# RmSchaffert/ACCV-Lab

Measured on AMD Instinct MI355X. Metric: heatmap frames/sec (1920x1080 fp32, ragged N_obj in [1,128], fused clear+draw), higher is better.
Workload: dtype f32

## Files before the change

accv-lab_amd/csrc/draw_heatmap.hip:

```cpp
#include <hip/hip_runtime.h>
#include <hip/hip_ext.h>

#include <algorithm>
#include <atomic>
#include <climits>
#include <cstdint>
#include <cstring>
#include <type_traits>

#include "accv_common.h"
#include "polyline_arith.h"

namespace {

constexpr int kWavesPerGroup = 1;
constexpr int kBoxTileR = 8;
constexpr int kCand = 64;
constexpr float kLog2e = 1.4426950408889634f;

struct SplatParams {
    float* hm;
    const int32_t* centers;
    const int32_t* radii;
    const int32_t* labels;
    const void* counts;
    const int32_t* plane_off;
    int H, W;
    int n_max;
    int n_classes;
    int tiles_x, tiles_y;
    long long n_tiles;
    float factor, k;
    int counts_i64;
    int grid3d;
    float dense_area;
    const float* centers_f;
    const float* boxes_f;
    float stride;
    int radius, n_groups;
};

constexpr int kMaxScales = 4;
struct MultiParams {
    SplatParams scale[kMaxScales];
    long long tile_begin[kMaxScales + 1];
    int n_scales;
};

struct __attribute__((aligned(16))) Hit {
    int x, y;
    float c2;
    unsigned box;
};

template <int PX>
struct Vec;
typedef float vfloat4 __attribute__((ext_vector_type(4)));
template <>
struct Vec<4> {
    using type = vfloat4;
};
template <>
struct Vec<1> {
    using type = float;
};

__device__ __forceinline__ float raw_exp2(float x) { return __builtin_amdgcn_exp2f(x); }

__device__ __forceinline__ float max_skip_nan(float acc, float v)
{
    float r;
    asm("v_max_f32 %0, %1, %2" : "=v"(r) : "v"(acc), "v"(v));
    return r;
}

struct TileCtx {
    int tx0, ty0, tx1, ty1;
    long long plane;
    const int2* centers2;
    const int32_t* radii;
    const int32_t* labels;
    const float2* centers_f;
    const float4* boxes_f;
    float4 box0;
    float stride;
    int radius;
    int n, cls;
};

template <bool SCALAR_COUNT = false>
__device__ __forceinline__ void plane_objects(const SplatParams& p, TileCtx& t);

template <int TW, int TH, int WPG, bool SCALAR_COUNT = false>
__device__ __forceinline__ bool locate_tile(const SplatParams& p, int wave, TileCtx& t, long long linear_group)
{
    int tx, ty;
    if (p.grid3d) {
        tx = blockIdx.x * WPG + wave;
        ty = blockIdx.y;
        t.plane = blockIdx.z;
        if (tx >= p.tiles_x) return false;
    } else {
        const long long tile = linear_group * WPG + wave;
        if (tile >= p.n_tiles) return false;
        if (p.n_tiles <= 0x7fffffffll) {
            const unsigned t32 = (unsigned)tile, t2 = t32 / (unsigned)p.tiles_x;
            tx = (int)(t32 - t2 * (unsigned)p.tiles_x);
            const unsigned pl = t2 / (unsigned)p.tiles_y;
            ty = (int)(t2 - pl * (unsigned)p.tiles_y);
            t.plane = pl;
        } else {
            tx = (int)(tile % p.tiles_x);
            const long long t2 = tile / p.tiles_x;
            ty = (int)(t2 % p.tiles_y);
            t.plane = t2 / p.tiles_y;
        }
    }
    t.tx0 = tx * TW;
    t.ty0 = ty * TH;
    t.tx1 = min(t.tx0 + TW, p.W);
    t.ty1 = min(t.ty0 + TH, p.H);
    plane_objects<SCALAR_COUNT>(p, t);
    return true;
}

template <bool SCALAR_COUNT>
__device__ __forceinline__ void plane_objects(const SplatParams& p, TileCtx& t)
{
    long long obj_base;
    t.cls = -1;
    if (p.plane_off) {
        const int o0 = p.plane_off[t.plane];
        obj_base = o0;
        t.n = p.plane_off[t.plane + 1] - o0;
    } else {
        long long s = t.plane;
        if (p.n_classes > 0) {
            s = t.plane / p.n_classes;
            t.cls = (int)(t.plane - s * p.n_classes);
        }
        long long cnt;
        if constexpr (SCALAR_COUNT) {
            if (p.n_groups > 0)
                t.box0 = reinterpret_cast<const float4*>(p.boxes_f)[t.plane * p.n_groups + min((int)(threadIdx.x & 63), p.n_groups - 1)];
            using ConstI32 = const __attribute__((address_space(4))) int;
            using ConstI64 = const __attribute__((address_space(4))) long long;
            const uintptr_t base = reinterpret_cast<uintptr_t>(p.counts);
            cnt = p.counts_i64 ? reinterpret_cast<ConstI64*>(base)[s] : (long long)reinterpret_cast<ConstI32*>(base)[s];
        } else {
            cnt = p.counts_i64 ? ((const long long*)p.counts)[s] : (long long)((const int*)p.counts)[s];
        }
        t.n = (int)max(0ll, min(cnt, (long long)p.n_max));
        obj_base = s * p.n_max;
    }
    t.centers2 = reinterpret_cast<const int2*>(p.centers) + obj_base;
    t.radii = p.radii + obj_base;
    t.labels = p.labels + obj_base;
    t.centers_f = reinterpret_cast<const float2*>(p.centers_f) + obj_base;
    t.boxes_f = reinterpret_cast<const float4*>(p.boxes_f) + (p.n_groups > 0 ? (t.plane * p.n_groups) : obj_base);
    t.stride = p.stride;
    t.radius = p.radius;
}

struct Cand {
    int x, y, r, label;
};
template <int SRC = 0>
__device__ __forceinline__ Cand cull_load(const TileCtx& t, int base, int lane)
{
    const int cc = min(base + lane, t.n - 1);
    if constexpr (SRC == 1) {
        const float2 c = t.centers_f[cc];
        const float4 b = t.boxes_f[cc];
        const float m = fminf(fminf(c.x - b.x, c.y - b.y), fminf(b.z - c.x, b.w - c.y));
        const bool pow2 = (__float_as_uint(t.stride) & 0x007fffffu) == 0u && t.stride > 1.0e-30f && t.stride < 1.0e30f;
        if (pow2) {
            const float inv = 1.0f / t.stride;
            int r = (int)ceilf(m * inv);
            if (r < 1) r = 1;
            return Cand{(int)(c.x * inv), (int)(c.y * inv), r, 0};
        }
        int r = (int)ceilf(__fdiv_rn(m, t.stride));
        if (r < 1) r = 1;
        return Cand{(int)__fdiv_rn(c.x, t.stride), (int)__fdiv_rn(c.y, t.stride), r, 0};
    } else if constexpr (SRC == 2) {
        const float2 c = t.centers_f[cc];
        const bool bad = (c.x != c.x) || (c.y != c.y);
        if (bad) return Cand{0, 0, -1, 0};
        return Cand{(int)__fdiv_rn(c.x, t.stride), (int)__fdiv_rn(c.y, t.stride), t.radius, 0};
    } else {
        const int2 cxy = t.centers2[cc];
        return Cand{cxy.x, cxy.y, t.radii[cc], t.labels[cc]};
    }
}
__device__ __forceinline__ unsigned long long cull_test(const TileCtx& t, int base, int lane, const Cand& c)
{
    constexpr int kClampXY = 1 << 29, kClampR = 1 << 30;
    const int xc = min(max(c.x, -kClampXY), kClampXY), yc = min(max(c.y, -kClampXY), kClampXY);
    const int rc = min(c.r, kClampR);
    const bool hit = (base + lane < t.n) && (t.cls < 0 || c.label == t.cls) && c.r >= 0 && xc - rc < t.tx1 &&
                     xc + rc >= t.tx0 && yc - rc < t.ty1 && yc + rc >= t.ty0;
    return __ballot(hit);
}
template <int SRC = 0>
__device__ __forceinline__ unsigned long long cull_round(const TileCtx& t, int base, int lane, int& x, int& y, int& r)
{
    const Cand c = cull_load<SRC>(t, base, lane);
    x = c.x;
    y = c.y;
    r = c.r;
    return cull_test(t, base, lane, c);
}

__device__ __forceinline__ float hit_exponent_scale(const SplatParams& p, int r)
{
    const float sigma = (float)(2 * r + 1) / p.factor;
    return kLog2e / (2.0f * sigma * sigma);
}
__device__ __forceinline__ Hit make_hit(const SplatParams& p, const TileCtx& t, int x, int y, int r, float c2);
__device__ __forceinline__ Hit make_hit(const SplatParams& p, const TileCtx& t, int x, int y, int r)
{
    return make_hit(p, t, x, y, r, hit_exponent_scale(p, r));
}
__device__ __forceinline__ Hit make_hit(const SplatParams& p, const TileCtx& t, int x, int y, int r, float c2)
{
    const long long x0 = (long long)x - min(x, r), x1 = (long long)x + min((long long)p.W - x, (long long)r + 1);
    const long long y0 = (long long)y - min(y, r), y1 = (long long)y + min((long long)p.H - y, (long long)r + 1);
    const long long xlo = max(x0, (long long)t.tx0) - t.tx0, xhi = min(x1, (long long)t.tx1) - t.tx0;
    const long long ylo = max(y0, (long long)t.ty0) - t.ty0, yhi = min(y1, (long long)t.ty1) - t.ty0;
    unsigned box = 0;
    if (xhi > xlo && yhi > ylo) box = (unsigned)xlo | ((unsigned)xhi << 8) | ((unsigned)ylo << 16) | ((unsigned)yhi << 24);
    return Hit{x, y, c2, box};
}

__device__ __forceinline__ float max3_skip_nan(float acc, float a, float b)
{
    float r;
    asm("v_max3_f32 %0, %1, %2, %3" : "=v"(r) : "v"(acc), "v"(a), "v"(b));
    return r;
}

template <int PX, int R, bool CLEAR, int SM, int WPG, int SRC>
__device__ __forceinline__ void splat_body(const SplatParams& p, long long linear_group)
{
    constexpr int kWavesPerGroup = WPG;
    constexpr int TW = 32 * PX;
    constexpr int TH = 2 * R;
    static_assert(R % 4 == 0, "row registers are fetched four at a time");

    __shared__ Hit s_hit[kWavesPerGroup][kCand];
    __shared__ __attribute__((aligned(16))) float s_ey[kWavesPerGroup][kCand][TH];

    const int lane = threadIdx.x & 63;
    const int wave = __builtin_amdgcn_readfirstlane(threadIdx.x >> 6);
    TileCtx t;
    if (!locate_tile<TW, TH, kWavesPerGroup>(p, wave, t, linear_group)) return;
    const int tx0 = t.tx0, ty0 = t.ty0, n = t.n;
    const long long plane = t.plane;

    const int sub = lane >> 5;
    const int col0 = tx0 + (lane & 31) * PX;

    float acc[R][PX];
    const float init = CLEAR ? 0.0f : __builtin_nanf("");
#pragma unroll
    for (int i = 0; i < R; ++i)
#pragma unroll
        for (int c = 0; c < PX; ++c) acc[i][c] = init;

    int total_hits = 0;
    float cover = 0.0f;

    for (int base = 0; base < n; base += kCand) {
        int x, y, r;
        const unsigned long long m = cull_round<SRC>(t, base, lane, x, y, r);
        if constexpr (SM == 5) {
            const float dia = (float)(2 * min(max(r, 0), 1 << 20) + 1);
            cover += (base + lane < n) ? dia * dia : 0.0f;
        }
        const bool hit = (m >> lane) & 1ull;
        const int nh = __popcll(m);
        if (nh == 0) continue;
        if constexpr (!CLEAR) {
            if (total_hits == 0 && col0 < p.W) {
                const float* plane_rd = p.hm + (size_t)plane * (size_t)p.H * (size_t)p.W;
#pragma unroll
                for (int i = 0; i < R; ++i) {
                    const int row = ty0 + sub * R + i;
                    if (row < p.H) {
                        if constexpr (PX == 4) {
                            const vfloat4 o = *reinterpret_cast<const vfloat4*>(plane_rd + (size_t)row * p.W + col0);
                            acc[i][0] = o.x;
                            acc[i][1] = o.y;
                            acc[i][2] = o.z;
                            acc[i][3] = o.w;
                        } else {
                            acc[i][0] = plane_rd[(size_t)row * p.W + col0];
                        }
                    }
                }
            }
        }
        if (hit) s_hit[wave][__popcll(m & ((1ull << lane) - 1ull))] = make_hit(p, t, x, y, r);
        __builtin_amdgcn_fence(__ATOMIC_RELEASE, "wavefront");
        __builtin_amdgcn_fence(__ATOMIC_ACQUIRE, "wavefront");

        for (int t = lane; t < nh * TH; t += 64) {
            const int h = t / TH, rr = t % TH;
            const Hit hy = s_hit[wave][h];
            const float d = (float)(ty0 + rr - hy.y);
            const float v = p.k * raw_exp2(-(d * d) * hy.c2);
            const unsigned ylo = (hy.box >> 16) & 255u, yhi = hy.box >> 24;
            s_ey[wave][h][rr] = ((unsigned)rr >= ylo && (unsigned)rr < yhi) ? v : __builtin_nanf("");
        }
        __builtin_amdgcn_fence(__ATOMIC_RELEASE, "wavefront");
        __builtin_amdgcn_fence(__ATOMIC_ACQUIRE, "wavefront");

        const unsigned colr0 = (unsigned)(lane & 31) * PX;
        auto column_factors = [&](const Hit& hx, float (&ex)[PX]) {
            const unsigned xlo = hx.box & 255u, xhi = (hx.box >> 8) & 255u;
#pragma unroll
            for (int c = 0; c < PX; ++c) {
                const float d = (float)(col0 + c - hx.x);
                const float e = raw_exp2(-(d * d) * hx.c2);
                ex[c] = (colr0 + c >= xlo && colr0 + c < xhi) ? e : __builtin_nanf("");
            }
        };
        int h = 0;
        for (; CLEAR && h + 1 < nh; h += 2) {
            float exa[PX], exb[PX];
            column_factors(s_hit[wave][h], exa);
            column_factors(s_hit[wave][h + 1], exb);
#pragma unroll
            for (int q = 0; q < R / 4; ++q) {
                const float4 a4 = *reinterpret_cast<const float4*>(&s_ey[wave][h][sub * R + 4 * q]);
                const float4 b4 = *reinterpret_cast<const float4*>(&s_ey[wave][h + 1][sub * R + 4 * q]);
                const float eya[4] = {a4.x, a4.y, a4.z, a4.w}, eyb[4] = {b4.x, b4.y, b4.z, b4.w};
#pragma unroll
                for (int i = 0; i < 4; ++i)
#pragma unroll
                    for (int c = 0; c < PX; ++c)
                        acc[4 * q + i][c] = max3_skip_nan(acc[4 * q + i][c], exa[c] * eya[i], exb[c] * eyb[i]);
            }
        }
        for (; h < nh; ++h) {
            float ex[PX];
            column_factors(s_hit[wave][h], ex);
#pragma unroll
            for (int q = 0; q < R / 4; ++q) {
                const float4 e4 = *reinterpret_cast<const float4*>(&s_ey[wave][h][sub * R + 4 * q]);
                const float ey[4] = {e4.x, e4.y, e4.z, e4.w};
#pragma unroll
                for (int i = 0; i < 4; ++i)
#pragma unroll
                    for (int c = 0; c < PX; ++c) acc[4 * q + i][c] = max_skip_nan(acc[4 * q + i][c], ex[c] * ey[i]);
            }
        }
        total_hits += nh;
        __builtin_amdgcn_fence(__ATOMIC_RELEASE, "wavefront");
        __builtin_amdgcn_fence(__ATOMIC_ACQUIRE, "wavefront");
    }

    if (!CLEAR && total_hits == 0) return;
    if (col0 >= p.W) return;

    using V = typename Vec<PX>::type;
    float* plane_ptr = p.hm + (size_t)plane * (size_t)p.H * (size_t)p.W;
    bool write_through = SM == 4;
    if constexpr (SM == 5 && PX == 4) {
#pragma unroll
        for (int d = 32; d >= 1; d >>= 1) cover += __shfl_xor(cover, d);
        write_through = cover >= p.dense_area;
    }
#pragma unroll
    for (int i = 0; i < R; ++i) {
        const int row = ty0 + sub * R + i;
        if (row >= p.H) break;
        V* dst = reinterpret_cast<V*>(plane_ptr + (size_t)row * p.W + col0);
        V out;
        if constexpr (PX == 4)
            out = V{acc[i][0], acc[i][1], acc[i][2], acc[i][3]};
        else
            out = acc[i][0];
        if constexpr (SM >= 4 && PX == 4) {
            if (write_through) {
                const auto rsrc = __builtin_amdgcn_make_buffer_rsrc(plane_ptr, 0, (int)((size_t)p.H * p.W * 4), 0x00020000);
                __builtin_amdgcn_raw_buffer_store_b128(out, rsrc, (int)(((size_t)row * p.W + col0) * 4), 0, 18);
            } else {
                *dst = out;
            }
        } else {
            *dst = out;
        }
    }
}

template <int PX, int R, bool CLEAR, int SM, int WPG = kWavesPerGroup>
__global__ __launch_bounds__(WPG * 64) void splat_kernel(const SplatParams p)
{
    splat_body<PX, R, CLEAR, SM, WPG, 0>(p, blockIdx.x);
}

__device__ __forceinline__ int scale_of_group(const MultiParams& mp, long long group, long long& first)
{
    int s = 0;
    first = 0;
#pragma unroll
    for (int i = 1; i < kMaxScales; ++i) {
        const long long begin = mp.tile_begin[i];
        if (group >= begin) {
            s = i;
            first = begin;
        }
    }
    return s;
}
template <typename T>
__device__ __forceinline__ void pin_scalar(T& v)
{
    asm volatile("" : "+s"(v));
}
__device__ __forceinline__ SplatParams preload_params(const SplatParams& src)
{
    SplatParams p = src;
    asm volatile("" ::"s"(p.hm), "s"(p.counts), "s"(p.centers_f), "s"(p.boxes_f));
    pin_scalar(p.H);
    pin_scalar(p.W);
    pin_scalar(p.n_max);
    pin_scalar(p.n_classes);
    pin_scalar(p.tiles_x);
    pin_scalar(p.tiles_y);
    pin_scalar(p.n_tiles);
    pin_scalar(p.factor);
    pin_scalar(p.k);
    pin_scalar(p.counts_i64);
    pin_scalar(p.grid3d);
    pin_scalar(p.dense_area);
    pin_scalar(p.stride);
    pin_scalar(p.radius);
    pin_scalar(p.n_groups);
    return p;
}

template <bool CLEAR, int SM>
__global__ __launch_bounds__(64) void splat_multi_kernel(const MultiParams mp)
{
    long long first;
    const int s = scale_of_group(mp, blockIdx.x, first);
    splat_body<4, kBoxTileR, CLEAR, SM, 1, 1>(mp.scale[s], (long long)blockIdx.x - first);
}

constexpr int kSmallTW = 128, kSmallTH = 16;
constexpr int kSmallLdsW = kSmallTW + 4;
using SmallTile = float (*)[kSmallLdsW];

template <bool WG_SCOPE>
__device__ __forceinline__ void walk_hits(const SplatParams& p, const TileCtx& t, int lane, int nh, const Hit* __restrict__ hits,
                                          SmallTile tile, int rows_hint)
{
    __builtin_amdgcn_fence(__ATOMIC_RELEASE, "wavefront");
    __builtin_amdgcn_fence(__ATOMIC_ACQUIRE, "wavefront");
    if (rows_hint > 0 && rows_hint <= 7) {
        const int per_pass = 64 / rows_hint;
        const int hl = (int)((float)lane * (1.0f / (float)rows_hint) + 1e-3f);
        const int rl = lane - hl * rows_hint;
        for (int h0 = 0; h0 < nh; h0 += per_pass) {
            const int h = h0 + hl;
            if (h >= nh || hl >= per_pass) continue;
            const Hit hh = hits[h];
            const int xlo = hh.box & 255u, xhi = (hh.box >> 8) & 255u, ylo = (hh.box >> 16) & 255u, yhi = hh.box >> 24;
            const int py = ylo + rl;
            if (py >= yhi) continue;
            const float dy = (float)(t.ty0 + py - hh.y);
            const float dy2 = dy * dy;
            float* row = &tile[py][0];
            for (int px = xlo; px < xhi; ++px) {
                const float dx = (float)(t.tx0 + px - hh.x);
                const float v = p.k * raw_exp2(-(dx * dx + dy2) * hh.c2);
                __hip_atomic_fetch_max(row + px, v, __ATOMIC_RELAXED,
                                       WG_SCOPE ? __HIP_MEMORY_SCOPE_WORKGROUP : __HIP_MEMORY_SCOPE_WAVEFRONT);
            }
        }
    } else {
        const int grp = lane >> 4, l16 = lane & 15;
        for (int h0 = 0; h0 < nh; h0 += 4) {
            const int h = h0 + grp;
            if (h >= nh) continue;
            const Hit hh = hits[h];
            const int xlo = hh.box & 255u, xhi = (hh.box >> 8) & 255u, ylo = (hh.box >> 16) & 255u, yhi = hh.box >> 24;
            const int w = xhi - xlo, area = w * (yhi - ylo);
            const float inv_w = 1.0f / (float)max(w, 1);
            for (int q = l16; q < area; q += 16) {
                const int py = (int)(((float)q + 0.5f) * inv_w);
                const int px = q - py * w;
                const float dx = (float)(t.tx0 + xlo + px - hh.x), dy = (float)(t.ty0 + ylo + py - hh.y);
                const float v = p.k * raw_exp2(-(dx * dx + dy * dy) * hh.c2);
                __hip_atomic_fetch_max(&tile[ylo + py][xlo + px], v, __ATOMIC_RELAXED,
                                       WG_SCOPE ? __HIP_MEMORY_SCOPE_WORKGROUP : __HIP_MEMORY_SCOPE_WAVEFRONT);
            }
        }
    }
    __builtin_amdgcn_fence(__ATOMIC_RELEASE, "wavefront");
    __builtin_amdgcn_fence(__ATOMIC_ACQUIRE, "wavefront");
}
template <bool WG_SCOPE>
__device__ __forceinline__ int splat_round(const SplatParams& p, const TileCtx& t, int lane, unsigned long long m, const Cand& cand,
                                           Hit* __restrict__ hits, SmallTile tile, int rows_hint = 0)
{
    const int nh = __popcll(m);
    int rows = 0;
    if ((m >> lane) & 1ull) {
        const Hit mine = make_hit(p, t, cand.x, cand.y, cand.r);
        hits[__popcll(m & ((1ull << lane) - 1ull))] = mine;
        rows = (int)(mine.box >> 24) - (int)((mine.box >> 16) & 255u);
    }
    if (rows_hint == 0) {
#pragma unroll
        for (int d = 32; d >= 1; d >>= 1) rows = max(rows, __shfl_xor(rows, d));
        rows_hint = max(1, __builtin_amdgcn_readfirstlane(rows));
    }
    walk_hits<WG_SCOPE>(p, t, lane, nh, hits, tile, rows_hint);
    return nh;
}

struct GroupBox {
    float x0, y0, x1, y1;
    bool valid;
};
template <bool FIRST = false>
__device__ __forceinline__ GroupBox load_group_box(const SplatParams& p, const TileCtx& t, int g)
{
    float4 v = FIRST ? t.box0 : t.boxes_f[min(g, p.n_groups - 1)];
    asm volatile("" : "+v"(v.x), "+v"(v.y), "+v"(v.z), "+v"(v.w));
    return GroupBox{v.x, v.y, v.z, v.w, g < p.n_groups && g * kCand < t.n && v.x <= v.z};
}
struct ReachBounds {
    float xlo, xhi, ylo, yhi;
};
__device__ __forceinline__ ReachBounds reach_bounds(const TileCtx& t, int rc, int cx0, int cx1, int cy0, int cy1)
{
    const float r1 = (float)min(rc, 1 << 24) + 2.0f;
    return ReachBounds{((float)cx0 - r1) * t.stride, ((float)cx1 + r1) * t.stride, ((float)cy0 - r1) * t.stride,
                       ((float)cy1 + r1) * t.stride};
}
__device__ __forceinline__ bool group_reaches(const GroupBox& b, const ReachBounds& rb)
{
    return b.valid && b.x1 >= rb.xlo && b.x0 < rb.xhi && b.y1 >= rb.ylo && b.y0 < rb.yhi;
}

constexpr int kDppQuad0 = 0x00, kDppQuad1 = 0x55, kDppQuad2 = 0xAA, kDppQuad3 = 0xFF;
constexpr int kDppRowShr = 0x110;
constexpr int kDppWaveShl1 = 0x130, kDppWaveShr1 = 0x138;
template <int CTRL>
__device__ __forceinline__ float dpp_f(float old, float src)
{
    return __int_as_float(__builtin_amdgcn_update_dpp(__float_as_int(old), __float_as_int(src), CTRL, 0xf, 0xf, false));
}
template <int CTRL>
__device__ __forceinline__ int dpp_i(int old, int src)
{
    return __builtin_amdgcn_update_dpp(old, src, CTRL, 0xf, 0xf, false);
}
__device__ __forceinline__ float2 request_group_samples(const TileCtx& t, int sub_base, int lane)
{
    return t.centers_f[min(sub_base + lane, t.n - 1)];
}
struct PixelScale {
    float stride, inv;
    bool pow2;
};
__device__ __forceinline__ PixelScale pixel_scale(float stride)
{
    const bool pow2 = (__float_as_uint(stride) & 0x007fffffu) == 0u && stride > 1.0e-30f && stride < 1.0e30f;
    return PixelScale{stride, pow2 ? 1.0f / stride : 0.0f, pow2};
}
__device__ __forceinline__ float to_pixels(float x, const PixelScale& ps) { return ps.pow2 ? x * ps.inv : __fdiv_rn(x, ps.stride); }
__device__ __forceinline__ Cand group_candidates(const TileCtx& t, const PixelScale& ps, const float2 c, int lane)
{
    Cand out{(int)to_pixels(c.x, ps), (int)to_pixels(c.y, ps), t.radius, 0};
    if ((c.x != c.x) || (c.y != c.y)) out = Cand{0, 0, -1, 0};
    const int nx = dpp_i<kDppWaveShr1>(0, out.x), ny = dpp_i<kDppWaveShr1>(0, out.y), nr = dpp_i<kDppWaveShr1>(-2, out.r);
    if (lane > 0 && nx == out.x && ny == out.y && nr == out.r) out.r = -1;
    return out;
}

template <int SM>
__device__ __forceinline__ void store_segment(const SplatParams& p, float* plane_ptr, int row, int col0, const vfloat4& v)
{
    if constexpr (SM == 4) {
        const auto rsrc = __builtin_amdgcn_make_buffer_rsrc(plane_ptr, 0, (int)((size_t)p.H * p.W * 4), 0x00020000);
        __builtin_amdgcn_raw_buffer_store_b128(v, rsrc, (int)(((size_t)row * p.W + col0) * 4), 0, 18);
    } else {
        *reinterpret_cast<vfloat4*>(plane_ptr + (size_t)row * p.W + col0) = v;
    }
}

template <bool CLEAR, int SM, int RPW>
__device__ __forceinline__ void write_back_rows(const SplatParams& p, const TileCtx& t, float* plane_ptr, SmallTile tile, int row0,
                                                int lane, int col0)
{
    const float init = CLEAR ? 0.0f : -__builtin_inff();
    constexpr int kBatch = RPW > 4 ? 4 : RPW;
    static_assert(RPW % kBatch == 0, "rows per half-wave come in whole batches");
#pragma unroll
    for (int i0 = 0; i0 < RPW; i0 += kBatch) {
        vfloat4 out[kBatch];
#pragma unroll
        for (int i = 0; i < kBatch; ++i) out[i] = *reinterpret_cast<const vfloat4*>(&tile[row0 + i0 + i][(lane & 31) * 4]);
        if constexpr (CLEAR) {
#pragma unroll
            for (int i = 0; i < kBatch; ++i) {
                const int row = t.ty0 + row0 + i0 + i;
                if (row < p.H) store_segment<SM>(p, plane_ptr, row, col0, out[i]);
            }
        } else {
            bool dirty[kBatch];
            vfloat4 old[kBatch];
#pragma unroll
            for (int i = 0; i < kBatch; ++i) {
                const int row = t.ty0 + row0 + i0 + i;
                dirty[i] = row < p.H && !(out[i].x == init && out[i].y == init && out[i].z == init && out[i].w == init);
                old[i] = vfloat4{0.0f, 0.0f, 0.0f, 0.0f};
                if (dirty[i]) old[i] = *reinterpret_cast<const vfloat4*>(plane_ptr + (size_t)row * p.W + col0);
            }
            const float nanv = __builtin_nanf("");
#pragma unroll
            for (int i = 0; i < kBatch; ++i) {
                if (!dirty[i]) continue;
                vfloat4 o = out[i];
                o.x = max_skip_nan(old[i].x, o.x == init ? nanv : o.x);
                o.y = max_skip_nan(old[i].y, o.y == init ? nanv : o.y);
                o.z = max_skip_nan(old[i].z, o.z == init ? nanv : o.z);
                o.w = max_skip_nan(old[i].w, o.w == init ? nanv : o.w);
                store_segment<SM>(p, plane_ptr, t.ty0 + row0 + i0 + i, col0, o);
            }
        }
    }
}

template <bool CLEAR, int SM, int SRC, int NW = 1, int TH = kSmallTH>
__device__ __forceinline__ void small_body(const SplatParams& p, long long linear_group, Hit (*s_hit)[kCand], SmallTile s_tile)
{
    constexpr int TW = kSmallTW;
    constexpr int RPW = TH / NW / 2;
    static_assert(TH % (2 * NW) == 0, "rows must split evenly over the half-waves of the workgroup");

    const int lane = threadIdx.x & 63;
    const int wave = NW > 1 ? __builtin_amdgcn_readfirstlane((int)threadIdx.x >> 6) : 0;
    TileCtx t;
    if (!locate_tile<TW, TH, 1, SRC == 2>(p, 0, t, linear_group)) return;
    const int sub = lane >> 5, col0 = t.tx0 + (lane & 31) * 4;
    const int row0 = wave * (TH / NW) + sub * RPW;
    float* plane_ptr = p.hm + (size_t)t.plane * (size_t)p.H * (size_t)p.W;

    const float init = CLEAR ? 0.0f : -__builtin_inff();
    vfloat4 vinit = vfloat4{init, init, init, init};
    asm volatile("" : "+v"(vinit));
    bool tile_ready = false;
    auto prepare_tile = [&]() {
        if (tile_ready) return;
        tile_ready = true;
#pragma unroll
        for (int i = 0; i < RPW; ++i) *reinterpret_cast<vfloat4*>(&s_tile[row0 + i][(lane & 31) * 4]) = vinit;
// ... 1275 lines not shown
```

Baseline: 711,000.

## Pack hits across cull rounds and share column exp factors via permlane32 swap

Restructures the splat loop for the clear path. Surviving hits from several cull rounds are gathered into one candidate list before accumulating, so there are fewer fence-separated passes. The two wave halves each compute column Gaussian factors for a different hit (or half the columns) and exchange them with permlane32_swap, which halves the exp2 work per lane. A 32-bit make_hit is used when a ballot shows no coordinate can overflow. This adds cross-lane shuffles and more complex control flow, and it only applies to the CLEAR, PX==4 configurations.

```diff
diff --git a/accv-lab_amd/csrc/draw_heatmap.hip b/accv-lab_amd/csrc/draw_heatmap.hip
--- a/accv-lab_amd/csrc/draw_heatmap.hip
+++ b/accv-lab_amd/csrc/draw_heatmap.hip
@@ -10,6 +10,19 @@
 
 #include "accv_common.h"
 #include "polyline_arith.h"
+
+#ifndef ACCV_SPLAT_ONE_LIST
+#define ACCV_SPLAT_ONE_LIST 1
+#endif
+#ifndef ACCV_SPLAT_SHARE_PAIR
+#define ACCV_SPLAT_SHARE_PAIR 1
+#endif
+#ifndef ACCV_SPLAT_HIT32
+#define ACCV_SPLAT_HIT32 1
+#endif
+#ifndef ACCV_SPLAT_SHARE_SINGLE
+#define ACCV_SPLAT_SHARE_SINGLE 1
+#endif
 
 namespace {
 
@@ -233,6 +246,17 @@
     return Hit{x, y, c2, box};
 }
 
+__device__ __forceinline__ Hit make_hit32(const SplatParams& p, const TileCtx& t, int x, int y, int r, float c2)
+{
+    const int x0 = x - min(x, r), x1 = x + min(p.W - x, r + 1);
+    const int y0 = y - min(y, r), y1 = y + min(p.H - y, r + 1);
+    const int xlo = max(x0, t.tx0) - t.tx0, xhi = min(x1, t.tx1) - t.tx0;
+    const int ylo = max(y0, t.ty0) - t.ty0, yhi = min(y1, t.ty1) - t.ty0;
+    unsigned box = 0;
+    if (xhi > xlo && yhi > ylo) box = (unsigned)xlo | ((unsigned)xhi << 8) | ((unsigned)ylo << 16) | ((unsigned)yhi << 24);
+    return Hit{x, y, c2, box};
+}
+
 __device__ __forceinline__ float max3_skip_nan(float acc, float a, float b)
 {
     float r;
@@ -247,6 +271,11 @@
     constexpr int TW = 32 * PX;
     constexpr int TH = 2 * R;
     static_assert(R % 4 == 0, "row registers are fetched four at a time");
+    constexpr bool ONE_LIST = CLEAR && PX == 4 && R == 16 && ACCV_SPLAT_ONE_LIST;
+    constexpr bool HIT32 = CLEAR && PX == 4 && ACCV_SPLAT_HIT32;
+    constexpr bool SHARE_PAIR = CLEAR && PX == 4 && ACCV_SPLAT_SHARE_PAIR;
+    constexpr bool SHARE_SINGLE = CLEAR && PX == 4 && SRC == 0 && ACCV_SPLAT_SHARE_SINGLE;
+    static_assert(!(ONE_LIST && SM == 5), "the cover sum of SM == 5 lives in the per-round loop");
 
     __shared__ Hit s_hit[kWavesPerGroup][kCand];
     __shared__ __attribute__((aligned(16))) float s_ey[kWavesPerGroup][kCand][TH];
@@ -271,40 +300,24 @@
     int total_hits = 0;
     float cover = 0.0f;
 
-    for (int base = 0; base < n; base += kCand) {
-        int x, y, r;
-        const unsigned long long m = cull_round<SRC>(t, base, lane, x, y, r);
-        if constexpr (SM == 5) {
-            const float dia = (float)(2 * min(max(r, 0), 1 << 20) + 1);
-            cover += (base + lane < n) ? dia * dia : 0.0f;
-        }
-        const bool hit = (m >> lane) & 1ull;
-        const int nh = __popcll(m);
-        if (nh == 0) continue;
-        if constexpr (!CLEAR) {
-            if (total_hits == 0 && col0 < p.W) {
-                const float* plane_rd = p.hm + (size_t)plane * (size_t)p.H * (size_t)p.W;
-#pragma unroll
-                for (int i = 0; i < R; ++i) {
-                    const int row = ty0 + sub * R + i;
-                    if (row < p.H) {
-                        if constexpr (PX == 4) {
-                            const vfloat4 o = *reinterpret_cast<const vfloat4*>(plane_rd + (size_t)row * p.W + col0);
-                            acc[i][0] = o.x;
-                            acc[i][1] = o.y;
-                            acc[i][2] = o.z;
-                            acc[i][3] = o.w;
-                        } else {
-                            acc[i][0] = plane_rd[(size_t)row * p.W + col0];
-                        }
-                    }
-                }
-            }
-        }
-        if (hit) s_hit[wave][__popcll(m & ((1ull << lane) - 1ull))] = make_hit(p, t, x, y, r);
+    const unsigned colr0 = (unsigned)(lane & 31) * PX;
+    auto column_factors = [&](const Hit& hx, auto& ex, int first) {
+        const unsigned xlo = hx.box & 255u, xhi = (hx.box >> 8) & 255u;
+#pragma unroll
+        for (int c = 0; c < (int)(sizeof(ex) / sizeof(float)); ++c) {
+            const float d = (float)(col0 + first + c - hx.x);
+            const float e = raw_exp2(-(d * d) * hx.c2);
+            ex[c] = (colr0 + first + c >= xlo && colr0 + first + c < xhi) ? e : __builtin_nanf("");
+        }
+    };
+    auto both_halves = [](float v, float& from_low, float& from_high) {
+        const auto sw = __builtin_amdgcn_permlane32_swap(__float_as_uint(v), __float_as_uint(v), false, false);
+        from_low = __uint_as_float(sw[0]);
+        from_high = __uint_as_float(sw[1]);
+    };
+    auto accumulate_list = [&](int nh) {
         __builtin_amdgcn_fence(__ATOMIC_RELEASE, "wavefront");
         __builtin_amdgcn_fence(__ATOMIC_ACQUIRE, "wavefront");
-
         for (int t = lane; t < nh * TH; t += 64) {
             const int h = t / TH, rr = t % TH;
             const Hit hy = s_hit[wave][h];
@@ -316,21 +329,18 @@
         __builtin_amdgcn_fence(__ATOMIC_RELEASE, "wavefront");
         __builtin_amdgcn_fence(__ATOMIC_ACQUIRE, "wavefront");
 
-        const unsigned colr0 = (unsigned)(lane & 31) * PX;
-        auto column_factors = [&](const Hit& hx, float (&ex)[PX]) {
-            const unsigned xlo = hx.box & 255u, xhi = (hx.box >> 8) & 255u;
-#pragma unroll
-            for (int c = 0; c < PX; ++c) {
-                const float d = (float)(col0 + c - hx.x);
-                const float e = raw_exp2(-(d * d) * hx.c2);
-                ex[c] = (colr0 + c >= xlo && colr0 + c < xhi) ? e : __builtin_nanf("");
-            }
-        };
         int h = 0;
         for (; CLEAR && h + 1 < nh; h += 2) {
             float exa[PX], exb[PX];
-            column_factors(s_hit[wave][h], exa);
-            column_factors(s_hit[wave][h + 1], exb);
+            if constexpr (SHARE_PAIR) {
+                float ex[PX];
+                column_factors(s_hit[wave][h + sub], ex, 0);
+#pragma unroll
+                for (int c = 0; c < PX; ++c) both_halves(ex[c], exa[c], exb[c]);
+            } else {
+                column_factors(s_hit[wave][h], exa, 0);
+                column_factors(s_hit[wave][h + 1], exb, 0);
+            }
 #pragma unroll
             for (int q = 0; q < R / 4; ++q) {
                 const float4 a4 = *reinterpret_cast<const float4*>(&s_ey[wave][h][sub * R + 4 * q]);
@@ -345,7 +355,14 @@
         }
         for (; h < nh; ++h) {
             float ex[PX];
-            column_factors(s_hit[wave][h], ex);
+            if constexpr (SHARE_SINGLE) {
+                float part[2];
+                column_factors(s_hit[wave][h], part, 2 * sub);
+                both_halves(part[0], ex[0], ex[2]);
+                both_halves(part[1], ex[1], ex[3]);
+            } else {
+                column_factors(s_hit[wave][h], ex, 0);
+            }
 #pragma unroll
             for (int q = 0; q < R / 4; ++q) {
                 const float4 e4 = *reinterpret_cast<const float4*>(&s_ey[wave][h][sub * R + 4 * q]);
@@ -356,9 +373,77 @@
                     for (int c = 0; c < PX; ++c) acc[4 * q + i][c] = max_skip_nan(acc[4 * q + i][c], ex[c] * ey[i]);
             }
         }
-        total_hits += nh;
         __builtin_amdgcn_fence(__ATOMIC_RELEASE, "wavefront");
         __builtin_amdgcn_fence(__ATOMIC_ACQUIRE, "wavefront");
+    };
+
+    auto write_hits = [&](unsigned long long m, int count, int x, int y, int r) {
+        const bool hit = (m >> lane) & 1ull;
+        const int slot = count + __popcll(m & ((1ull << lane) - 1ull));
+        if constexpr (HIT32) {
+            const bool wide = hit && ((unsigned)x + (1u << 29) > (1u << 30) || (unsigned)y + (1u << 29) > (1u << 30) ||
+                                      (unsigned)r > (1u << 30));
+            if (__ballot(wide) == 0ull) {
+                if (hit) s_hit[wave][slot] = make_hit32(p, t, x, y, r, hit_exponent_scale(p, r));
+                return;
+            }
+        }
+        if (hit) s_hit[wave][slot] = make_hit(p, t, x, y, r);
+    };
+
+    if constexpr (ONE_LIST) {
+        int base = 0, count = 0;
+        for (;;) {
+            while (base < n) {
+                int x, y, r;
+                const unsigned long long m = cull_round<SRC>(t, base, lane, x, y, r);
+                const int nh = __popcll(m);
+                if (count + nh > kCand) break;
+                base += kCand;
+                if (nh == 0) continue;
+                write_hits(m, count, x, y, r);
+                count += nh;
+            }
+            if (count == 0) break;
+            total_hits += count;
+            accumulate_list(count);
+            count = 0;
+            if (base >= n) break;
+        }
+    } else {
+        for (int base = 0; base < n; base += kCand) {
+            int x, y, r;
+            const unsigned long long m = cull_round<SRC>(t, base, lane, x, y, r);
+            if constexpr (SM == 5) {
+                const float dia = (float)(2 * min(max(r, 0), 1 << 20) + 1);
+                cover += (base + lane < n) ? dia * dia : 0.0f;
+            }
+            const int nh = __popcll(m);
+            if (nh == 0) continue;
+            if constexpr (!CLEAR) {
+                if (total_hits == 0 && col0 < p.W) {
+                    const float* plane_rd = p.hm + (size_t)plane * (size_t)p.H * (size_t)p.W;
+#pragma unroll
+                    for (int i = 0; i < R; ++i) {
+                        const int row = ty0 + sub * R + i;
+                        if (row < p.H) {
+                            if constexpr (PX == 4) {
+                                const vfloat4 o = *reinterpret_cast<const vfloat4*>(plane_rd + (size_t)row * p.W + col0);
+                                acc[i][0] = o.x;
+                                acc[i][1] = o.y;
+                                acc[i][2] = o.z;
+                                acc[i][3] = o.w;
+                            } else {
+                                acc[i][0] = plane_rd[(size_t)row * p.W + col0];
+                            }
+                        }
+                    }
+                }
+            }
+            write_hits(m, 0, x, y, r);
+            accumulate_list(nh);
+            total_hits += nh;
+        }
     }
 
     if (!CLEAR && total_hits == 0) return;
```

Result: no change. 718,000 (median of 6 runs) (+1.0%).
